# zkeown/mlx-audio-primitives

Measured on AMD Instinct MI355X. Metric: mel-spectrogram frames/sec (n_fft=2048, n_mels=128), higher is better.
Workload: dtype f32

## Files before the change

mlx-audio-primitives_amd/csrc/kernels_mel2048.h:

```cpp
#pragma once
#include <type_traits>
#include "kernels_wave.h"

#define APM_WAVES 8
#define APM_RUN 8
#define APM_PARTIAL_OFF 1152


#define APM_REG_WIN 1
#define APM_REG_TW1 2
#define APM_REG_TW2 4
#define APM_REG_SPLIT 8
#define APM_REGS (APM_REG_WIN | APM_REG_SPLIT)

template <int REGS>
AP_DEV void apm_forward(const ap_float2 (&x)[16], const ap_float2 (&w)[16], ap_float2 *X, const ap_float2 *TW1,
                        const ap_float2 *tw2row, const ap_float2 (&t1r)[16], const ap_float2 (&t2r)[16],
                        const ApwLane &c, const ApmLane &m) {
    const int lane = c.lane;
    ap_float2 v[16];
    if (REGS & APM_REG_TW1) {
        ApButterfly<16>::run_weighted(x, w, v);
#pragma unroll
        for (int k = 1; k < 16; ++k) v[k] = ap_mul_fw(v[k], t1r[k]);
    } else {
        ap_float2 t1[16];
#pragma unroll
        for (int k = 1; k < 16; ++k) t1[k] = TW1[k * 64 + lane];
        ApButterfly<16>::run_weighted(x, w, v);
#pragma unroll
        for (int k = 1; k < 16; ++k) v[k] = ap_mul_fw(v[k], t1[k]);
    }
    {
        const int a = lane & 3, bq = lane >> 2;
#pragma unroll
        for (int k = 0; k < 16; ++k) X[APW_T1(k * 4 + a) + bq] = v[k];
    }
    AP_WAVE_SYNC();
    ap_float2 t2[16];
#pragma unroll
    for (int i = 0; i < 16; ++i) v[i] = X[APW_T1(lane) + i];
    if (!(REGS & APM_REG_TW2)) {
#pragma unroll
        for (int cc = 1; cc < 16; ++cc) t2[cc] = tw2row[cc];
    }
    AP_WAVE_SYNC();
    ApButterfly<16>::run(v);
    v[0] = ap_scale(v[0], m.sg);
#pragma unroll
    for (int cc = 1; cc < 16; ++cc) v[cc] = ap_mul_fw(v[cc], (REGS & APM_REG_TW2) ? t2r[cc] : t2[cc]);
    apm_quad_radix4(v, m);
#pragma unroll
    for (int cc = 0; cc < 16; ++cc) X[apw_zidx(c.k1p + 16 * cc + 256 * c.qd)] = v[cc];
    AP_WAVE_SYNC();
}

template <int REGS>
AP_DEV void apm_split(const ap_float2 *X, const ApwLane &c, const ap_float2 (&wsp)[8], ap_float2 (&xk)[8],
                      ap_float2 (&xm)[8], ap_float2 &zh) {
    ap_float2 zk[8], zm[8];
#pragma unroll
    for (int r = 0; r < 8; ++r) {
        const int k = c.lane + 64 * r;
        zk[r] = X[apw_zidx(k)];
        zm[r] = X[apw_zidx((APW_NC - k) & (APW_NC - 1))];
    }
    zh = X[apw_zidx(APW_NC / 2)];
    AP_WAVE_SYNC();
#pragma unroll
    for (int r = 0; r < 8; ++r) {
        const ap_float2 a = ap_add_conj(zk[r], zm[r]);
        const ap_float2 d = ap_sub_conj(zk[r], zm[r]);
        const ap_float2 w = (REGS & APM_REG_SPLIT) ? wsp[r]
                                                   : (r == 0 ? c.tws0h : ap_mul_bw_c(c.tws0h, APW_C32(r), APW_S32(r)));
        const ap_float2 u = ap_mul_fw(d, w);
        xk[r] = ap_fma_add_mi(a, c.half, u);
        xm[r] = ap_fma_sub_mi(a, c.half, u);
    }
}

#ifdef AP_DIAG_STAMPS
#define AP_DIAG_BEGIN() unsigned long long ap_dt0, ap_dr0; \
    asm volatile("s_memtime %0\n\ts_memrealtime %1\n\ts_waitcnt lgkmcnt(0)" : "=s"(ap_dt0), "=s"(ap_dr0)::"memory")
#define AP_DIAG_END(widx) do { unsigned long long ap_dt1, ap_dr1; \
    asm volatile("s_memtime %0\n\ts_memrealtime %1\n\ts_waitcnt lgkmcnt(0)" : "=s"(ap_dt1), "=s"(ap_dr1)::"memory"); \
    if ((threadIdx.x & 63) == 0 && (widx) < 256 * 16) { ap_diag_stamps[4 * (widx)] = ap_dt1 - ap_dt0; ap_diag_stamps[4 * (widx) + 1] = ap_dr1 - ap_dr0; ap_diag_stamps[4 * (widx) + 2] = ap_dr0; ap_diag_stamps[4 * (widx) + 3] = ap_dr1; } } while (0)
#else
#define AP_DIAG_BEGIN() do {} while (0)
#define AP_DIAG_END(widx) do {} while (0)
#endif

#ifdef AP_HOST_EMU
#define AP_FAIR_SHARE(wave, nw, f) do {} while (0)
#else
#define AP_FAIR_SHARE(wave, nw, f)                                   \
    do {                                                             \
        if ((wave) >= (nw) / 2 + ((nw) > 8 ? 2 : 0)) {               \
            if ((f) & 1) __builtin_amdgcn_s_setprio(1);              \
            else __builtin_amdgcn_s_setprio(0);                      \
        } else if ((nw) > 8 && (wave) >= 4) {                        \
            if ((f) & 1) __builtin_amdgcn_s_setprio(0);              \
            else __builtin_amdgcn_s_setprio(1);                      \
        }                                                            \
    } while (0)
#endif

template <int PMODE, int NPASS, int HOPJ, int IN16 = 0, int NW = APM_WAVES, int REGS = APM_REGS>
__global__ void __launch_bounds__(64 * NW, NW / 4) ap_mel2048_run_kernel(ApMelWaveParams P) {
    static_assert(IN16 != 1 || (REGS & APM_REG_WIN), "the PCM scale rides on the register-resident window");
    const int tid = threadIdx.x;
    const int lane = tid & 63;
    const int wave = AP_UNIFORM(tid >> 6);
    ap_float2 *X = reinterpret_cast<ap_float2 *>(ap_smem) + wave * APW_X_COMPLEX;
    ap_float2 *TW2 = reinterpret_cast<ap_float2 *>(ap_smem + P.off_tw2);
    const ap_float2 *TW1 = reinterpret_cast<const ap_float2 *>(ap_smem + P.off_tw1);
    const ap_float2 *WIN = reinterpret_cast<const ap_float2 *>(ap_smem + P.off_win);
    const ap_float4 *WQ = reinterpret_cast<const ap_float4 *>(ap_smem + P.off_wq);
    float *pp = reinterpret_cast<float *>(X);
    float *partial = pp + APM_PARTIAL_OFF;
    const int M = P.n_mels;

    {
        const int nt = 64 * NW;
        ap_float4 *wq = reinterpret_cast<ap_float4 *>(ap_smem + P.off_wq);
        for (int i = tid; i < P.n_quads; i += nt) wq[i] = reinterpret_cast<const ap_float4 *>(P.quads)[i];
        apw_fill_tables(TW2, reinterpret_cast<ap_float2 *>(ap_smem + P.off_tw1),
                        reinterpret_cast<ap_float2 *>(ap_smem + P.off_win), P.tw, P.window, tid, nt);
    }
    AP_LDS_BARRIER();
    const ApwLane lc = apw_lane_init(lane, TW2, P.tw);
    const ApmLane lm = apm_lane_init(lane);
    ap_float2 winr[16], t1r[16], t2r[16], wsp[8];
#pragma unroll
    for (int j = 0; j < 16; ++j) {
        winr[j] = (REGS & APM_REG_WIN) ? reinterpret_cast<const ap_float2 *>(P.window)[lane + 64 * j] : ap_mk(0.0f, 0.0f);
        if (IN16 == 1) winr[j] = ap_scale(winr[j], 1.0f / 32768.0f);
        t1r[j] = (REGS & APM_REG_TW1) ? P.tw[(2 * lane * j) & 2047] : ap_mk(0.0f, 0.0f);
        t2r[j] = (REGS & APM_REG_TW2) ? ap_scale(P.tw[32 * (lane & 3) * j], lm.sg) : ap_mk(0.0f, 0.0f);
    }
#pragma unroll
    for (int r = 0; r < 8; ++r)
        wsp[r] = (REGS & APM_REG_SPLIT) ? ap_scale(P.tw[lane + 64 * r], 0.5f) : ap_mk(0.0f, 0.0f);
    const ap_float4 *pqa[NPASS], *pqb[NPASS];
    float *sa[NPASS], *sb[NPASS];
    float fz[NPASS];
#pragma unroll
    for (int ps = 0; ps < NPASS; ++ps) {
        const int pi = lane + 64 * ps;
        ap_int4 pd;
        pd.x = P.n_slots; pd.y = 0; pd.z = P.n_slots; pd.w = 0;
        if (pi < P.n_parts) pd = reinterpret_cast<const ap_int4 *>(P.parts)[pi];
        pqa[ps] = reinterpret_cast<const ap_float4 *>(pp) + pd.y;
        pqb[ps] = reinterpret_cast<const ap_float4 *>(pp) + pd.w;
        sa[ps] = partial + pd.x;
        sb[ps] = partial + (pd.z < 0 ? P.n_slots : pd.z);
        fz[ps] = pd.z < 0 ? 1.0f : 0.0f;
    }
    int rs0[2], cnt[2];
#pragma unroll
    for (int i = 0; i < 2; ++i) {
        const int row = lane + 64 * i;
        rs0[i] = row < M ? P.rowstart[row] : 0;
        cnt[i] = row < M ? P.rowstart[row + 1] - rs0[i] : 0;
    }
    AP_LDS_BARRIER();

    const int64_t worker = (int64_t)blockIdx.x * NW + wave;
    const int64_t n_workers = (int64_t)gridDim.x * NW;
    const int64_t n_frames = P.n_clips * P.T;
    const int64_t f_lo = n_frames * worker / n_workers, f_hi = n_frames * (worker + 1) / n_workers;
    const int Ti = (int)P.T;
    float vmax = -INFINITY;
    AP_DIAG_BEGIN();
    if (f_lo < f_hi) {
        int64_t b = f_lo / P.T;
        int t = (int)(f_lo - b * P.T);
        const int16_t *y16 = reinterpret_cast<const int16_t *>(P.y);
        ApClip clip = ap_clip_make(P.y + (IN16 == 1 ? 0 : b * P.L), IN16 == 1 ? 0 : P.L);
        ApClip16 clip16 = ap_clip16_make(y16 + (IN16 == 1 ? b * P.L : 0), IN16 == 1 ? P.L : 0);
        auto ld2 = [&](int64_t bb, int base, int p) -> ap_float2 {
            if (IN16 == 1) return ap_clip16_load2(clip16, p);
            if (IN16 == 2 && !(base >= 0 && (int64_t)base + 2 * APW_NC <= P.L)) {
                const float *yb = P.y + bb * P.L;
                return ap_mk(ap_load_padded(yb, P.L, p, P.pad_mode), ap_load_padded(yb, P.L, p + 1, P.pad_mode));
            }
            return ap_clip_load2(clip, p);
        };
        constexpr int U = HOPJ == 4 ? 4 : 1;
        ap_float2 raw[16];
        auto load_frame = [&](int tt, auto rot_tag) {
            constexpr int ROT = decltype(rot_tag)::value;
            const int base = tt * P.hop - P.pad;
#pragma unroll
            for (int j = 0; j < 16; ++j) {
                const int p = base + 2 * (lane + 64 * j);
                raw[(j + HOPJ * ROT) & 15] = ld2(b, base, p);
            }
        };
        const int r0 = U == 4 ? (t & 3) : 0;
        if (r0 == 1) load_frame(t, std::integral_constant<int, 1 % U>());
        else if (r0 == 2) load_frame(t, std::integral_constant<int, 2 % U>());
        else if (r0 == 3) load_frame(t, std::integral_constant<int, 3 % U>());
        else load_frame(t, std::integral_constant<int, 0>());
        float acc0[APM_RUN], acc1[APM_RUN];
#pragma unroll
        for (int i = 0; i < APM_RUN; ++i) { acc0[i] = 0.0f; acc1[i] = 0.0f; }
        int nrun = 0, half = U == 4 ? ((t >> 2) & 1) : 0;
        int64_t f = f_lo;

        auto frame = [&](auto rot_tag) -> bool {
            constexpr int ROT = decltype(rot_tag)::value;
            constexpr int NROT = (ROT + 1) % U;
            AP_FAIR_SHARE(wave, NW, f);
            const bool clip_ends = t + 1 == Ti;
            const bool more = f + 1 < f_hi;
            {
                ap_float2 xs[16], ws[16];
#pragma unroll
                for (int j = 0; j < 16; ++j) xs[j] = raw[(j + HOPJ * ROT) & 15];
                if (REGS & APM_REG_WIN) {
#pragma unroll
                    for (int j = 0; j < 16; ++j) ws[j] = winr[j];
                } else {
#pragma unroll
                    for (int j = 0; j < 16; ++j) ws[j] = WIN[lane + 64 * j];
                }
                AP_SCHED_FENCE();
                apm_forward<REGS>(xs, ws, X, TW1, lc.tw2row, t1r, t2r, lc, lm);
            }
            AP_SCHED_FENCE();
            if (more) {
                if (clip_ends) {
                    if (IN16 == 1) clip16 = ap_clip16_make(y16 + (b + 1) * P.L, P.L);
                    else clip = ap_clip_make(P.y + (b + 1) * P.L, P.L);
                }
                const int base = (clip_ends ? 0 : t + 1) * P.hop - P.pad;
#pragma unroll
                for (int j = 16 - HOPJ; j < 16; ++j) {
                    const int p = base + 2 * (lane + 64 * j);
                    raw[(j + HOPJ * NROT) & 15] = ld2(clip_ends ? b + 1 : b, base, p);
                }
                if (HOPJ == 0 || clip_ends) {
#pragma unroll
                    for (int j = 0; j < 16 - HOPJ; ++j) {
                        const int p = base + 2 * (lane + 64 * j);
                        raw[(j + HOPJ * NROT) & 15] = ld2(clip_ends ? b + 1 : b, base, p);
                    }
                }
            }
            AP_SCHED_FENCE();
            {
                ap_float2 xk[8], xm[8], zh;
                apm_split<REGS>(X, lc, wsp, xk, xm, zh);
#pragma unroll
                for (int r = 0; r < 8; ++r) {
                    const int k = lane + 64 * r;
                    pp[k] = apw_pow2x<PMODE>(xk[r].x, xk[r].y, P.power);
                    pp[APW_NC - k] = apw_pow2x<PMODE>(xm[r].x, xm[r].y, P.power);
                }
                if (lane == 0) pp[APW_NC / 2] = apw_pow2x<PMODE>(zh.x, zh.y, P.power);
            }
            AP_WAVE_SYNC();
#pragma unroll
            for (int ps = 0; ps < NPASS; ++ps) {
                const ap_float4 *wq = WQ + 256 * ps + lane;
                ap_float4 w[4], q[4];
#pragma unroll
                for (int i = 0; i < 4; ++i) w[i] = wq[64 * i];
                q[0] = pqa[ps][0]; q[1] = pqa[ps][1]; q[2] = pqb[ps][0]; q[3] = pqb[ps][1];
                float acc[2] = {0.0f, 0.0f};
#pragma unroll
                for (int i = 0; i < 4; ++i) {
                    acc[i >> 1] = fmaf(w[i].x, q[i].x, acc[i >> 1]);
                    acc[i >> 1] = fmaf(w[i].y, q[i].y, acc[i >> 1]);
                    acc[i >> 1] = fmaf(w[i].z, q[i].z, acc[i >> 1]);
                    acc[i >> 1] = fmaf(w[i].w, q[i].w, acc[i >> 1]);
                }
                *sa[ps] = fmaf(fz[ps], acc[1], acc[0]);
                *sb[ps] = acc[1];
            }
            AP_WAVE_SYNC();
            float sum2[2];
#pragma unroll
            for (int i = 0; i < 2; ++i) {
                const float p0 = partial[rs0[i]], p1 = partial[rs0[i] + 1], p2 = partial[rs0[i] + 2],
                            p3 = partial[rs0[i] + 3];
                float sum = cnt[i] > 0 ? p0 : 0.0f;
                sum += cnt[i] > 1 ? p1 : 0.0f;
                sum += cnt[i] > 2 ? p2 : 0.0f;
                sum += cnt[i] > 3 ? p3 : 0.0f;
                sum2[i] = sum;
                vmax = fmaxf(vmax, cnt[i] > 0 ? sum : vmax);
            }
            int pos;
            if (U == 1) {
#pragma unroll
                for (int i = 0; i < APM_RUN - 1; ++i) { acc0[i] = acc0[i + 1]; acc1[i] = acc1[i + 1]; }
                acc0[APM_RUN - 1] = sum2[0];
                acc1[APM_RUN - 1] = sum2[1];
                pos = APM_RUN - 1;
            } else {
                if (half) { acc0[4 + ROT] = sum2[0]; acc1[4 + ROT] = sum2[1]; }
                else { acc0[ROT] = sum2[0]; acc1[ROT] = sum2[1]; }
                pos = 4 * half + ROT;
            }
            ++nrun;
            AP_WAVE_SYNC();
            if ((U == 1 ? nrun == APM_RUN : pos == APM_RUN - 1) || clip_ends || !more) {
                const int first = pos - nrun + 1;
                float *ob = P.out + b * (int64_t)M * P.Ts + (t - nrun + 1);
#pragma unroll
                for (int i = 0; i < 2; ++i) {
                    const int row = lane + 64 * i;
                    if (row < M) {
                        float *dst = ob + (int64_t)row * P.Ts;
                        const float *src = i == 0 ? acc0 : acc1;
                        if (nrun == APM_RUN) {
                            ap_rsp_f4u lo, hi;
                            lo.x = src[0]; lo.y = src[1]; lo.z = src[2]; lo.w = src[3];
                            hi.x = src[4]; hi.y = src[5]; hi.z = src[6]; hi.w = src[7];
                            *reinterpret_cast<ap_rsp_f4u *>(dst) = lo;
                            *reinterpret_cast<ap_rsp_f4u *>(dst + 4) = hi;
                        } else {
#pragma unroll
                            for (int g = 0; g < APM_RUN; ++g)
                                if (g >= first && g <= pos) dst[g - first] = src[g];
                        }
                    }
                }
                nrun = 0;
            }
            if (clip_ends) { t = 0; ++b; } else { ++t; }
            ++f;
            return more;
        };
        if (U == 1) {
            while (frame(std::integral_constant<int, 0>())) {}
        } else {
            int skip = r0;
            for (;;) {
                if (skip <= 0 && !frame(std::integral_constant<int, 0>())) break;
                if (skip <= 1 && !frame(std::integral_constant<int, 1 % U>())) break;
                if (skip <= 2 && !frame(std::integral_constant<int, 2 % U>())) break;
                if (!frame(std::integral_constant<int, 3 % U>())) break;
                skip = 0;
                half ^= 1;
            }
        }
    }
    AP_DIAG_END((int)worker);
    if (P.max_key) {
        AP_WAVE_SYNC();
        partial[lane] = vmax;
        AP_WAVE_SYNC();
        if (lane == 0) {
            float m = partial[0];
            for (int i = 1; i < 64; ++i) m = fmaxf(m, partial[i]);
            ap_atomic_max_u32(P.max_key, ap_fkey(m));
        }
    }
}

#ifdef AP_HOST_EMU
AP_DEV float apm_lane_xor(float x, int mask) { return emu_lane_xor(x, mask); }
AP_DEV float apm_lane_up(float x, int d, int lane) { return emu_lane_perm(x, lane - d); }
#else
AP_DEV float apm_lane_xor(float x, int mask) { return __shfl_xor(x, mask, 64); }
AP_DEV float apm_lane_up(float x, int d, int lane) { return __shfl_up(x, d, 64); }
#endif
AP_DEV float apm_wave_sum(float x) {
#pragma unroll
    for (int off = 32; off > 0; off >>= 1) x += apm_lane_xor(x, off);
    return x;
}

template <int PMODE, int HOPJ, int FLAT, int PGEN = 0, int NW = APM_WAVES, int REGS = APM_REGS>
__global__ void __launch_bounds__(64 * NW, NW / 4) ap_spec2048_run_kernel(ApSpecWaveParams P) {
    const int tid = threadIdx.x;
    const int lane = tid & 63;
    const int wave = AP_UNIFORM(tid >> 6);
    ap_float2 *X = reinterpret_cast<ap_float2 *>(ap_smem) + wave * APW_X_COMPLEX;
    ap_float2 *TW2 = reinterpret_cast<ap_float2 *>(ap_smem + P.off_tw2);
    const ap_float2 *TW1 = reinterpret_cast<const ap_float2 *>(ap_smem + P.off_tw1);
    const ap_float2 *WIN = reinterpret_cast<const ap_float2 *>(ap_smem + P.off_win);
    float *pp = reinterpret_cast<float *>(X);
    apw_fill_tables(TW2, reinterpret_cast<ap_float2 *>(ap_smem + P.off_tw1),
                    reinterpret_cast<ap_float2 *>(ap_smem + P.off_win), P.tw, P.window, tid, 64 * NW);
    AP_LDS_BARRIER();
    const ApwLane lc = apw_lane_init(lane, TW2, P.tw);
    const ApmLane lm = apm_lane_init(lane);
    ap_float2 winr[16], t1r[16], t2r[16], wsp[8];
#pragma unroll
    for (int j = 0; j < 16; ++j) {
        winr[j] = (REGS & APM_REG_WIN) ? reinterpret_cast<const ap_float2 *>(P.window)[lane + 64 * j] : ap_mk(0.0f, 0.0f);
        t1r[j] = (REGS & APM_REG_TW1) ? P.tw[(2 * lane * j) & 2047] : ap_mk(0.0f, 0.0f);
        t2r[j] = (REGS & APM_REG_TW2) ? ap_scale(P.tw[32 * (lane & 3) * j], lm.sg) : ap_mk(0.0f, 0.0f);
    }
#pragma unroll
    for (int r = 0; r < 8; ++r)
        wsp[r] = (REGS & APM_REG_SPLIT) ? ap_scale(P.tw[lane + 64 * r], 0.5f) : ap_mk(0.0f, 0.0f);
    float fk[17];
#pragma unroll
    for (int i = 0; i < 16; ++i) fk[i] = P.freq[16 * lane + i];
    fk[16] = lane == 63 ? P.freq[APW_NC] : 0.0f;
    AP_LDS_BARRIER();

    const int64_t worker = (int64_t)blockIdx.x * NW + wave;
    const int64_t n_workers = (int64_t)gridDim.x * NW;
    const int64_t n_frames = P.n_clips * P.T;
    const int64_t f_lo = n_frames * worker / n_workers, f_hi = n_frames * (worker + 1) / n_workers;
    const int Ti = (int)P.T;
    if (f_lo >= f_hi) return;
    int64_t b = f_lo / P.T;
    int t = (int)(f_lo - b * P.T);
    ApClip clip = ap_clip_make(P.y + b * P.L, P.L);
    constexpr int U = HOPJ == 4 ? 4 : 1;
    ap_float2 raw[16];
    auto load_frame = [&](int tt, auto rot_tag) {
        constexpr int ROT = decltype(rot_tag)::value;
        const int base = tt * P.hop - P.pad;
#pragma unroll
        for (int j = 0; j < 16; ++j) raw[(j + HOPJ * ROT) & 15] = ap_clip_load2(clip, base + 2 * (lane + 64 * j));
    };
    load_frame(t, std::integral_constant<int, 0>());
    int64_t f = f_lo;
    const float F_all = (float)(APW_NC + 1);

    auto frame = [&](auto rot_tag) -> bool {
        constexpr int ROT = decltype(rot_tag)::value;
        constexpr int NROT = (ROT + 1) % U;
        const bool clip_ends = t + 1 == Ti;
        const bool more = f + 1 < f_hi;
        {
            ap_float2 xs[16], ws[16];
#pragma unroll
            for (int j = 0; j < 16; ++j) xs[j] = raw[(j + HOPJ * ROT) & 15];
            if (REGS & APM_REG_WIN) {
#pragma unroll
                for (int j = 0; j < 16; ++j) ws[j] = winr[j];
            } else {
#pragma unroll
                for (int j = 0; j < 16; ++j) ws[j] = WIN[lane + 64 * j];
            }
            AP_SCHED_FENCE();
            apm_forward<REGS>(xs, ws, X, TW1, lc.tw2row, t1r, t2r, lc, lm);
        }
        AP_SCHED_FENCE();
        if (more) {
            if (clip_ends) clip = ap_clip_make(P.y + (b + 1) * P.L, P.L);
            const int base = (clip_ends ? 0 : t + 1) * P.hop - P.pad;
#pragma unroll
            for (int j = 16 - HOPJ; j < 16; ++j)
                raw[(j + HOPJ * NROT) & 15] = ap_clip_load2(clip, base + 2 * (lane + 64 * j));
            if (HOPJ == 0 || clip_ends) {
#pragma unroll
                for (int j = 0; j < 16 - HOPJ; ++j)
                    raw[(j + HOPJ * NROT) & 15] = ap_clip_load2(clip, base + 2 * (lane + 64 * j));
            }
        }
        AP_SCHED_FENCE();
        {
            ap_float2 xk[8], xm[8], zh;
            apm_split<REGS>(X, lc, wsp, xk, xm, zh);
#pragma unroll
            for (int r = 0; r < 8; ++r) {
                const int k = lane + 64 * r;
                pp[k] = apw_pow2x<PMODE>(xk[r].x, xk[r].y, P.power);
                pp[APW_NC - k] = apw_pow2x<PMODE>(xm[r].x, xm[r].y, P.power);
            }
            if (lane == 0) pp[APW_NC / 2] = apw_pow2x<PMODE>(zh.x, zh.y, P.power);
        }
        AP_WAVE_SYNC();
        float v[17];
#pragma unroll
        for (int q4 = 0; q4 < 4; ++q4) {
            const ap_float4 a = reinterpret_cast<const ap_float4 *>(pp)[4 * lane + q4];
            v[4 * q4] = a.x; v[4 * q4 + 1] = a.y; v[4 * q4 + 2] = a.z; v[4 * q4 + 3] = a.w;
        }
        v[16] = lane == 63 ? pp[APW_NC] : 0.0f;
        AP_WAVE_SYNC();
        float s0 = 0.0f, s1 = 0.0f;
#pragma unroll
        for (int i = 0; i < 17; ++i) { s0 += v[i]; s1 = fmaf(fk[i], v[i], s1); }
        const float tot = apm_wave_sum(s0), tf = apm_wave_sum(s1);
        const float cen = tf / (tot + 1e-10f);
        const int64_t o = b * P.T + t;
        if (P.centroid && lane == 0) P.centroid[o] = cen;
        if (FLAT) {
            float sl = 0.0f, sa = 0.0f;
#pragma unroll
            for (int i = 0; i < 17; ++i) {
                const float c = fmaxf(v[i], P.amin);
                if (i < 16 || lane == 63) { sl += logf(c); sa += c; }
            }
            const float tl = apm_wave_sum(sl), ta = apm_wave_sum(sa);
            if (P.flatness && lane == 0) P.flatness[o] = expf(tl / F_all) / (ta / F_all + 1e-10f);
        }
        if (P.bandwidth) {
            float dev = 0.0f;
#pragma unroll
            for (int i = 0; i < 17; ++i) {
                const float d = fabsf(fk[i] - cen);
                dev = fmaf(v[i], PGEN ? powf(d, P.p) : d * d, dev);
            }
            float w = apm_wave_sum(dev);
            if (P.norm) w = w / (tot + 1e-10f);
            if (lane == 0) P.bandwidth[o] = PGEN ? powf(w, 1.0f / P.p) : sqrtf(w);
        }
        if (P.rolloff) {
            float incl = s0;
#pragma unroll
            for (int d = 1; d < 64; d <<= 1) {
                const float up = apm_lane_up(incl, d, lane);
                if (lane >= d) incl += up;
            }
            const float before = incl - s0;
            const float thr = tot * P.roll_percent;
            const bool mine = (before + s0 >= thr) && (lane == 0 || before < thr);
            float run = before, fsel = lane == 63 ? fk[16] : fk[15];
            bool found = false;
#pragma unroll
            for (int i = 0; i < 17; ++i) {
                if (i < 16 || lane == 63) {
                    run += v[i];
                    if (!found && run >= thr) { found = true; fsel = fk[i]; }
                }
            }
            float cand = (mine && found) ? fsel : INFINITY;
#pragma unroll
            for (int off = 32; off > 0; off >>= 1) cand = fminf(cand, apm_lane_xor(cand, off));
            const float last = apm_lane_xor(fk[16], 63);
            if (lane == 0) P.rolloff[o] = !(tot >= thr) ? fk[0] : (cand < INFINITY ? cand : last);
        }
        if (clip_ends) { t = 0; ++b; } else { ++t; }
        ++f;
        return more;
    };
    if (U == 1) {
        while (frame(std::integral_constant<int, 0>())) {}
    } else {
        for (;;) {
            if (!frame(std::integral_constant<int, 0>())) break;
            if (!frame(std::integral_constant<int, 1 % U>())) break;
            if (!frame(std::integral_constant<int, 2 % U>())) break;
            if (!frame(std::integral_constant<int, 3 % U>())) break;
        }
    }
}
```

mlx-audio-primitives_amd/csrc/kernels_wave.h:

```cpp
#pragma once
#include "ap_wave_params.h"
#include "fft_lds.h"
#include "kernels_generic.h"

#if defined(AP_DIAG_STAMPS) && !defined(AP_HOST_EMU)
__device__ unsigned long long ap_diag_stamps[4 * 256 * 16];
#endif

#define APW_C32(r) ((float)__builtin_cos(6.283185307179586476925 * (r) / 32.0))
#define APW_S32(r) ((float)__builtin_sin(6.283185307179586476925 * (r) / 32.0))

#ifdef AP_HOST_EMU
#define AP_WAVE_SYNC() emu_wave_sync()
#define AP_SCHED_FENCE() do {} while (0)
#define AP_PIN(x) do {} while (0)
#else
#define AP_SCHED_FENCE() __builtin_amdgcn_sched_barrier(0)
#define AP_PIN(x) asm volatile("" : "+v"(x))
#define AP_WAVE_SYNC()                                          \
    do {                                                        \
        __builtin_amdgcn_fence(__ATOMIC_RELEASE, "wavefront");  \
        __builtin_amdgcn_wave_barrier();                        \
        __builtin_amdgcn_fence(__ATOMIC_ACQUIRE, "wavefront");  \
    } while (0)

AP_DEV float ap_quad_xor1(float x) {
    return __builtin_bit_cast(float, __builtin_amdgcn_mov_dpp(__builtin_bit_cast(int, x), 0xB1, 0xF, 0xF, true));
}
AP_DEV float ap_quad_xor2(float x) {
    return __builtin_bit_cast(float, __builtin_amdgcn_mov_dpp(__builtin_bit_cast(int, x), 0x4E, 0xF, 0xF, true));
}
#endif


AP_DEV int apw_zidx(int k) { return k + 4 * (k >> 8); }

template <int PMODE>
AP_DEV float apw_pow2x(float re, float im, float power) {
    const float p2 = re * re + im * im;
    if (PMODE == 2) return p2;
    if (PMODE == 1) return sqrtf(p2);
    return powf(sqrtf(p2), power);
}

#ifdef AP_HOST_EMU
#define AP_UNIFORM(x) (x)
struct ApClip { const float *base; int64_t n; };
AP_DEV ApClip ap_clip_make(const float *base, int64_t n) { ApClip c; c.base = base; c.n = n; return c; }
AP_DEV float ap_clip_load(const ApClip &c, int64_t idx) { return (idx >= 0 && idx < c.n) ? c.base[idx] : 0.0f; }
AP_DEV ap_float2 ap_clip_load2(const ApClip &c, int64_t idx) { return ap_mk(ap_clip_load(c, idx), ap_clip_load(c, idx + 1)); }
struct ApClip16 { const int16_t *base; int64_t n; };
AP_DEV ApClip16 ap_clip16_make(const int16_t *base, int64_t n) { ApClip16 c; c.base = base; c.n = n; return c; }
AP_DEV ap_float2 ap_clip16_load2(const ApClip16 &c, int64_t idx) {
    return ap_mk((idx >= 0 && idx < c.n) ? (float)c.base[idx] : 0.0f,
                 (idx + 1 >= 0 && idx + 1 < c.n) ? (float)c.base[idx + 1] : 0.0f);
}
struct ApOutBuf { char *base; int64_t bytes; };
AP_DEV ApOutBuf ap_outbuf_make(void *base, int64_t bytes) { ApOutBuf o; o.base = (char *)base; o.bytes = bytes; return o; }
AP_DEV ap_float2 ap_outbuf_load2(const ApOutBuf &o, unsigned lane_bytes, unsigned uniform_bytes) {
    const uint64_t off = (uint64_t)lane_bytes + uniform_bytes;
    if (lane_bytes < 0x80000000u && off + 8 <= (uint64_t)o.bytes) return *reinterpret_cast<const ap_float2 *>(o.base + off);
    return ap_mk(0.0f, 0.0f);
}
AP_DEV void ap_outbuf_store2(const ApOutBuf &o, unsigned lane_bytes, unsigned uniform_bytes, ap_float2 v) {
    const uint64_t off = (uint64_t)lane_bytes + uniform_bytes;
    if (lane_bytes < 0x80000000u && off + 8 <= (uint64_t)o.bytes) *reinterpret_cast<ap_float2 *>(o.base + off) = v;
}
#else
#define AP_UNIFORM(x) __builtin_amdgcn_readfirstlane(x)
typedef __amdgpu_buffer_rsrc_t ApClip;
AP_DEV ApClip ap_clip_make(const float *base, int64_t n) {
    return __builtin_amdgcn_make_buffer_rsrc(const_cast<float *>(base), 0, (int)(n * 4), 0x00020000);
}
AP_DEV float ap_clip_load(ApClip c, int64_t idx) {
    int off = (int)(idx * 4);
    AP_PIN(off);
    return __builtin_bit_cast(float, __builtin_amdgcn_raw_buffer_load_b32(c, off, 0, 0));
}
AP_DEV ap_float2 ap_clip_load2(ApClip c, int idx) {
    typedef int ap_i2 __attribute__((ext_vector_type(2)));
    return __builtin_bit_cast(ap_float2, __builtin_bit_cast(ap_i2, __builtin_amdgcn_raw_buffer_load_b64(c, idx * 4, 0, 0)));
}
typedef __amdgpu_buffer_rsrc_t ApOutBuf;
AP_DEV ApOutBuf ap_outbuf_make(void *base, int64_t bytes) {
    return __builtin_amdgcn_make_buffer_rsrc(base, 0, (int)bytes, 0x00020000);
}
AP_DEV ap_float2 ap_outbuf_load2(ApOutBuf o, unsigned lane_bytes, unsigned uniform_bytes) {
    typedef int ap_i2 __attribute__((ext_vector_type(2)));
    return __builtin_bit_cast(ap_float2, __builtin_amdgcn_raw_buffer_load_b64(o, (int)lane_bytes, (int)uniform_bytes, 0));
}
AP_DEV void ap_outbuf_store2(ApOutBuf o, unsigned lane_bytes, unsigned uniform_bytes, ap_float2 v) {
    typedef int ap_i2 __attribute__((ext_vector_type(2)));
    __builtin_amdgcn_raw_buffer_store_b64(__builtin_bit_cast(ap_i2, v), o, (int)lane_bytes, (int)uniform_bytes, 0);
}
typedef __amdgpu_buffer_rsrc_t ApClip16;
AP_DEV ApClip16 ap_clip16_make(const int16_t *base, int64_t n) {
    return __builtin_amdgcn_make_buffer_rsrc(const_cast<int16_t *>(base), 0, (int)(n * 2), 0x00020000);
}
AP_DEV ap_float2 ap_clip16_load2(ApClip16 c, int idx) {
    int off = idx * 2;
    AP_PIN(off);
    const int d = __builtin_amdgcn_raw_buffer_load_b32(c, off, 0, 0);
    return ap_mk((float)(short)(d & 0xFFFF), (float)(d >> 16));
}
#endif


struct ApwLane {
    int lane, qa, qd, k1p;
    float s1, s2;
    ap_float2 rotw;
    const ap_float2 *tw2row;
    ap_float2 tws0h;
    ap_float2 half, halfc;
};

AP_DEV ApwLane apw_lane_init(int lane, const ap_float2 *TW2, const ap_float2 *tw) {
    ApwLane c;
    c.lane = lane;
    c.qa = lane & 3;
    c.s1 = c.qa < 2 ? 1.0f : -1.0f;
    c.s2 = (c.qa & 1) ? -1.0f : 1.0f;
    c.rotw = c.qa == 3 ? ap_mk(0.0f, 1.0f) : ap_mk(1.0f, 0.0f);
    c.qd = ((c.qa & 1) << 1) | (c.qa >> 1);
    c.k1p = lane >> 2;
    c.tw2row = TW2 + c.qa * 17;
    c.tws0h = ap_scale(tw[lane], 0.5f);
    c.half = ap_mk(0.5f, 0.5f);
    c.halfc = ap_mk(0.5f, -0.5f);
    return c;
}

AP_DEV void apw_fill_tables(ap_float2 *tw2, ap_float2 *tw1, ap_float2 *win, const ap_float2 *tw,
                            const float *window, int tid, int nt) {
    if (tid < 64) {
        const int a = tid >> 4;
        tw2[a * 17 + (tid & 15)] = ap_scale(tw[32 * a * (tid & 15)], (a == 1 || a == 2) ? -1.0f : 1.0f);
    }
    for (int i = tid; i < 16 * 64; i += nt) tw1[i] = tw[2 * (i & 63) * (i >> 6)];
    for (int i = tid; i < APW_NC; i += nt) win[i] = reinterpret_cast<const ap_float2 *>(window)[i];
}

struct ApmLane {
    float c1, c2;
    float sg;
    bool rot;
};

AP_DEV ApmLane apm_lane_init(int lane) {
    ApmLane m;
    const int qa = lane & 3;
    const float s1 = qa < 2 ? 1.0f : -1.0f, s2 = (qa & 1) ? -1.0f : 1.0f;
    m.c1 = -s1;
    m.c2 = -s2;
    m.sg = s1 * s2;
    m.rot = qa == 3;
    return m;
}

#ifdef AP_HOST_EMU
AP_DEV void apm_quad8(ap_float2 *v, const ApmLane &m) {
    for (int i = 0; i < 8; ++i) {
        v[i].x = v[i].x + m.c1 * ap_quad_xor2(v[i].x);
        v[i].y = v[i].y + m.c1 * ap_quad_xor2(v[i].y);
    }
    for (int i = 0; i < 8; ++i) {
        const float rx = v[i].x, ry = v[i].y;
        v[i].x = m.rot ? ry : rx;
        v[i].y = m.rot ? -rx : ry;
    }
    for (int i = 0; i < 8; ++i) {
        v[i].x = v[i].x + m.c2 * ap_quad_xor1(v[i].x);
        v[i].y = v[i].y + m.c2 * ap_quad_xor1(v[i].y);
    }
}
#else
#define APM_ROT(ix, iy, nx, ny)                            \
    "v_cndmask_b32 %" #nx ", %" #ix ", %" #iy ", %34\n\t"  \
    "v_cndmask_b32 %" #ny ", %" #iy ", -%" #ix ", %34\n\t"
#define APM_S2N(i) "v_fmac_f32_dpp %" #i ", %" #i ", %33 quad_perm:[1,0,3,2] row_mask:0xf bank_mask:0xf\n\t"
#define APM_S1N(i) "v_fmac_f32_dpp %" #i ", %" #i ", %32 quad_perm:[2,3,0,1] row_mask:0xf bank_mask:0xf\n\t"
AP_DEV void apm_quad8(ap_float2 *v, const ApmLane &m) {
    ap_float2 n[8];
    const unsigned long long rot_mask = 0x8888888888888888ull;
    asm volatile(
        "s_nop 1\n\t"
        APM_S1N(0) APM_S1N(1) APM_S1N(2) APM_S1N(3) APM_S1N(4) APM_S1N(5) APM_S1N(6) APM_S1N(7)
        APM_S1N(8) APM_S1N(9) APM_S1N(10) APM_S1N(11) APM_S1N(12) APM_S1N(13) APM_S1N(14) APM_S1N(15)
        APM_ROT(0, 1, 16, 17) APM_ROT(2, 3, 18, 19) APM_ROT(4, 5, 20, 21) APM_ROT(6, 7, 22, 23)
        APM_ROT(8, 9, 24, 25) APM_ROT(10, 11, 26, 27) APM_ROT(12, 13, 28, 29) APM_ROT(14, 15, 30, 31)
        APM_S2N(16) APM_S2N(17) APM_S2N(18) APM_S2N(19) APM_S2N(20) APM_S2N(21) APM_S2N(22) APM_S2N(23)
        APM_S2N(24) APM_S2N(25) APM_S2N(26) APM_S2N(27) APM_S2N(28) APM_S2N(29) APM_S2N(30) APM_S2N(31)
        : "+v"(v[0].x), "+v"(v[0].y), "+v"(v[1].x), "+v"(v[1].y), "+v"(v[2].x), "+v"(v[2].y), "+v"(v[3].x), "+v"(v[3].y),
          "+v"(v[4].x), "+v"(v[4].y), "+v"(v[5].x), "+v"(v[5].y), "+v"(v[6].x), "+v"(v[6].y), "+v"(v[7].x), "+v"(v[7].y),
          "=&v"(n[0].x), "=&v"(n[0].y), "=&v"(n[1].x), "=&v"(n[1].y), "=&v"(n[2].x), "=&v"(n[2].y), "=&v"(n[3].x), "=&v"(n[3].y),
          "=&v"(n[4].x), "=&v"(n[4].y), "=&v"(n[5].x), "=&v"(n[5].y), "=&v"(n[6].x), "=&v"(n[6].y), "=&v"(n[7].x), "=&v"(n[7].y)
        : "v"(m.c1), "v"(m.c2), "s"(rot_mask));
#pragma unroll
    for (int i = 0; i < 8; ++i) v[i] = n[i];
}
#undef APM_S1N
#undef APM_S2N
#undef APM_ROT
#endif

AP_DEV void apm_quad_radix4(ap_float2 (&v)[16], const ApmLane &m) {
    apm_quad8(&v[0], m);
    apm_quad8(&v[8], m);
}

AP_DEV void apw_butterfly16_tight(ap_float2 (&v)[16]) {
    ap_float2 a[4][4];
#pragma unroll
    for (int r = 0; r < 4; ++r) {
        a[r][0] = v[r]; a[r][1] = v[r + 4]; a[r][2] = v[r + 8]; a[r][3] = v[r + 12];
        ap_fft4(a[r][0], a[r][1], a[r][2], a[r][3]);
        AP_SCHED_FENCE();
    }
    const float C1 = 0.92387953251128675613f, S1 = 0.38268343236508977173f;
    const float H = 0.70710678118654752440f;
#pragma unroll
    for (int p = 0; p < 4; ++p) {
        if (p == 1) {
            a[1][1] = ap_mul_fw_c(a[1][1], C1, S1);
            a[2][1] = ap_mul_fw_c(a[2][1], H, H);
            a[3][1] = ap_mul_fw_c(a[3][1], S1, C1);
        } else if (p == 2) {
            a[1][2] = ap_mul_fw_c(a[1][2], H, H);
            a[3][2] = ap_mul_fw_c(a[3][2], -H, H);
        } else if (p == 3) {
            a[1][3] = ap_mul_fw_c(a[1][3], S1, C1);
            a[2][3] = ap_mul_fw_c(a[2][3], -H, H);
            a[3][3] = ap_mul_fw_c(a[3][3], -C1, -S1);
        }
        if (p == 2) ap_fft4_a2mi(a[0][p], a[1][p], a[2][p], a[3][p]);
        else ap_fft4(a[0][p], a[1][p], a[2][p], a[3][p]);
        v[p] = a[0][p]; v[p + 4] = a[1][p]; v[p + 8] = a[2][p]; v[p + 12] = a[3][p];
        AP_SCHED_FENCE();
    }
}

#ifndef AP_HOST_EMU
#define AP_PRIO(n) __builtin_amdgcn_s_setprio(n)
#else
#define AP_PRIO(n) do {} while (0)
#endif

template <bool TO_LDS = true, bool TIGHT = false, bool PRIO = false>
AP_DEV void apw_forward(ap_float2 (&v)[16], ap_float2 *X, const ap_float2 *TW1, const ApwLane &c) {
    const int lane = c.lane;
    if (TIGHT) {
        apw_butterfly16_tight(v);
#pragma unroll
        for (int h = 0; h < 2; ++h) {
            ap_float2 t1[8];
#pragma unroll
            for (int k = 0; k < 8; ++k) if (8 * h + k) t1[k] = TW1[(8 * h + k) * 64 + lane];
#pragma unroll
            for (int k = 0; k < 8; ++k) if (8 * h + k) v[8 * h + k] = ap_mul_fw(v[8 * h + k], t1[k]);
            AP_SCHED_FENCE();
        }
    } else {
        ap_float2 t1[16];
#pragma unroll
        for (int k = 1; k < 16; ++k) t1[k] = TW1[k * 64 + lane];
        ApButterfly<16>::run(v);
#pragma unroll
        for (int k = 1; k < 16; ++k) v[k] = ap_mul_fw(v[k], t1[k]);
    }
    if (PRIO) AP_PRIO(2);
    {
        const int a = lane & 3, bq = lane >> 2;
#pragma unroll
        for (int k = 0; k < 16; ++k) X[APW_T1(k * 4 + a) + bq] = v[k];
    }
    AP_WAVE_SYNC();
    ap_float2 t2[16];
#pragma unroll
    for (int i = 0; i < 16; ++i) v[i] = X[APW_T1(lane) + i];
    if (!TIGHT) {
#pragma unroll
        for (int cc = 1; cc < 16; ++cc) t2[cc] = c.tw2row[cc];
    }
    AP_WAVE_SYNC();
    const ApmLane m = apm_lane_init(lane);
    if (TIGHT) {
        AP_SCHED_FENCE();
        apw_butterfly16_tight(v);
        v[0] = ap_scale(v[0], m.sg);
#pragma unroll
        for (int h = 0; h < 2; ++h) {
#pragma unroll
            for (int k = 0; k < 8; ++k) if (8 * h + k) t2[k] = c.tw2row[8 * h + k];
#pragma unroll
            for (int k = 0; k < 8; ++k) if (8 * h + k) v[8 * h + k] = ap_mul_fw(v[8 * h + k], t2[k]);
            AP_SCHED_FENCE();
        }
    } else {
        ApButterfly<16>::run(v);
        v[0] = ap_scale(v[0], m.sg);
#pragma unroll
        for (int cc = 1; cc < 16; ++cc) v[cc] = ap_mul_fw(v[cc], t2[cc]);
    }
    if (PRIO) AP_PRIO(1);
    apm_quad_radix4(v, m);
    if (TO_LDS) {
#pragma unroll
        for (int cc = 0; cc < 16; ++cc) X[apw_zidx(c.k1p + 16 * cc + 256 * c.qd)] = v[cc];
        AP_WAVE_SYNC();
    }
}

template <bool CONJ>
AP_DEV void apw_split(const ap_float2 *X, const ApwLane &c, ap_float2 (&xk)[8], ap_float2 (&xm)[8],
                      ap_float2 &zh) {
    ap_float2 zk[8], zm[8];
#pragma unroll
    for (int r = 0; r < 8; ++r) {
        const int k = c.lane + 64 * r;
        zk[r] = X[apw_zidx(k)];
        zm[r] = X[apw_zidx((APW_NC - k) & (APW_NC - 1))];
    }
    zh = X[apw_zidx(APW_NC / 2)];
    AP_WAVE_SYNC();
#pragma unroll
    for (int r = 0; r < 8; ++r) {
        const ap_float2 a = ap_add_conj(zk[r], zm[r]);
        const ap_float2 d = ap_sub_conj(zk[r], zm[r]);
        const ap_float2 w = r == 0 ? c.tws0h : ap_mul_bw_c(c.tws0h, APW_C32(r), APW_S32(r));
        const ap_float2 u = ap_mul_fw(d, w);
        xk[r] = ap_fma_add_mi(a, c.half, u);
        xm[r] = CONJ ? ap_fma_sub_swap(a, c.halfc, u) : ap_fma_sub_mi(a, c.half, u);
    }
}

template <int PMODE, int PADGEN>
__global__ void __launch_bounds__(64 * APW_WAVES, 2) ap_mel2048_wave_kernel(ApMelWaveParams P) {
    const int tid = threadIdx.x;
    const int lane = tid & 63;
    const int wave = AP_UNIFORM(tid >> 6);
    ap_float2 *X = reinterpret_cast<ap_float2 *>(ap_smem) + wave * APW_X_COMPLEX;
    const ap_float2 *TW2 = reinterpret_cast<const ap_float2 *>(ap_smem + P.off_tw2);
    const ap_float2 *TW1 = reinterpret_cast<const ap_float2 *>(ap_smem + P.off_tw1);
    const ap_float2 *WIN = reinterpret_cast<const ap_float2 *>(ap_smem + P.off_win);
    const ap_float4 *WQ = reinterpret_cast<const ap_float4 *>(ap_smem + P.off_wq);
    const ap_int4 *PART = reinterpret_cast<const ap_int4 *>(ap_smem + P.off_parts);
    float *partial = reinterpret_cast<float *>(ap_smem + P.off_partial) + wave * P.partial_stride;
    float *otile = reinterpret_cast<float *>(ap_smem + P.off_otile) + wave * P.otile_stride * APW_G;
    const int M = P.n_mels;

    {
        const int nt = 64 * APW_WAVES;
        ap_float4 *wq = reinterpret_cast<ap_float4 *>(ap_smem + P.off_wq);
        ap_int4 *part = reinterpret_cast<ap_int4 *>(ap_smem + P.off_parts);
        for (int i = tid; i < P.n_quads; i += nt) wq[i] = reinterpret_cast<const ap_float4 *>(P.quads)[i];
        if (P.n_parts > 64 * APW_PASSES)
            for (int i = tid; i < P.n_parts; i += nt) part[i] = reinterpret_cast<const ap_int4 *>(P.parts)[i];
        apw_fill_tables(reinterpret_cast<ap_float2 *>(ap_smem + P.off_tw2),
                        reinterpret_cast<ap_float2 *>(ap_smem + P.off_tw1),
                        reinterpret_cast<ap_float2 *>(ap_smem + P.off_win), P.tw, P.window, tid, nt);
    }
    const ApwLane lc = apw_lane_init(lane, TW2, P.tw);
    float *pp = reinterpret_cast<float *>(X);
    ap_int4 mypart[APW_PASSES];
#pragma unroll
    for (int ps = 0; ps < APW_PASSES; ++ps) {
        const int pi = lane + 64 * ps;
        mypart[ps].x = 0; mypart[ps].y = 0; mypart[ps].z = 0; mypart[ps].w = 0;
        if (pi < P.n_parts) mypart[ps] = reinterpret_cast<const ap_int4 *>(P.parts)[pi];
    }
    int rs0[2], rs1[2];
#pragma unroll
    for (int i = 0; i < 2; ++i) {
        const int row = lane + 64 * i;
        rs0[i] = row < M ? P.rowstart[row] : 0;
        rs1[i] = row < M ? P.rowstart[row + 1] : 0;
    }
    AP_LDS_BARRIER();

    const int64_t worker = (int64_t)blockIdx.x * APW_WAVES + wave;
    const int64_t n_workers = (int64_t)gridDim.x * APW_WAVES;
    const int64_t n_frames = P.n_clips * P.T;
    const int64_t f_lo = n_frames * worker / n_workers, f_hi = n_frames * (worker + 1) / n_workers;
    float vmax = -INFINITY;
#ifdef AP_DIAG_STAMPS
    unsigned long long ap_dt0, ap_dr0;
    asm volatile("s_memtime %0\n\ts_memrealtime %1\n\ts_waitcnt lgkmcnt(0)" : "=s"(ap_dt0), "=s"(ap_dr0)::"memory");
#endif
    ap_float2 raw[16];
    auto load_frame = [&](int64_t f) {
        const int64_t b = f / P.T;
        const int64_t t = f - b * P.T;
        const float *yb = P.y + b * P.L;
        const ApClip clip = ap_clip_make(yb, P.L);
        const int64_t base = t * (int64_t)P.hop - P.pad;
        const bool inside = !PADGEN || (base >= 0 && base + 2 * APW_NC <= P.L);
        if (inside) {
#pragma unroll
            for (int j = 0; j < 16; ++j) {
                const int64_t p = base + 2 * (lane + 64 * j);
                raw[j] = ap_clip_load2(clip, (int)p);
            }
        } else {
#pragma unroll
            for (int j = 0; j < 16; ++j) {
                const int64_t p = base + 2 * (lane + 64 * j);
                raw[j] = ap_mk(ap_load_padded(yb, P.L, p, P.pad_mode), ap_load_padded(yb, P.L, p + 1, P.pad_mode));
            }
        }
    };
    auto next_frame = [&](int64_t f) {
        const int64_t b = f / P.T;
        const int64_t t = f - b * P.T;
        if (PADGEN || t == 0 || P.hopj == 0) { load_frame(f); return; }
        const ApClip clip = ap_clip_make(P.y + b * P.L, P.L);
        const int64_t base = t * (int64_t)P.hop - P.pad;
#define APW_SHIFT_LOAD(S)                                                                    \
        {                                                                                    \
            _Pragma("unroll") for (int j = 0; j < 16 - (S); ++j) raw[j] = raw[j + (S)];      \
            _Pragma("unroll") for (int j = 16 - (S); j < 16; ++j) {                           \
                const int64_t p = base + 2 * (lane + 64 * j);                                \
                raw[j] = ap_clip_load2(clip, (int)p);            \
            }                                                                                \
        }
        if (P.hopj == 4) APW_SHIFT_LOAD(4)
        else if (P.hopj == 2) APW_SHIFT_LOAD(2)
        else APW_SHIFT_LOAD(8)
#undef APW_SHIFT_LOAD
    };
    if (f_lo < f_hi) load_frame(f_lo);

    for (int64_t f = f_lo; f < f_hi;) {
        const int64_t b = f / P.T;
        const int64_t t0 = f - b * P.T;
        int64_t run = P.T - t0;
        if (run > APW_G) run = APW_G;
        if (run > f_hi - f) run = f_hi - f;
        const int Gt = (int)run;
        float *ob = P.out + b * (int64_t)M * P.T + t0;

// ... 460 lines not shown
```

Baseline: 586.9 million.

## Fold final radix-4 FFT stage into split via per-lane bin-pair mapping

Removes the cross-lane quad radix-4 stage and sign-scaled twiddles from the forward FFT. Stage-2 outputs are instead stored in a padded group layout, and each lane loads 4 float4 pairs, does local radix-4 butterflies, and directly owns conjugate bin pairs for the real-FFT split. Split twiddles are precomputed per lane from a packed lane-permutation table. The aim is to cut DPP/cross-lane work and use wider LDS reads, at the cost of more complex indexing and a possible change in bank-conflict behaviour.

```diff
diff --git a/mlx-audio-primitives_amd/csrc/kernels_mel2048.h b/mlx-audio-primitives_amd/csrc/kernels_mel2048.h
--- a/mlx-audio-primitives_amd/csrc/kernels_mel2048.h
+++ b/mlx-audio-primitives_amd/csrc/kernels_mel2048.h
@@ -5,7 +5,6 @@
 #define APM_WAVES 8
 #define APM_RUN 8
 #define APM_PARTIAL_OFF 1152
-
 
 #define APM_REG_WIN 1
 #define APM_REG_TW1 2
@@ -13,10 +12,30 @@
 #define APM_REG_SPLIT 8
 #define APM_REGS (APM_REG_WIN | APM_REG_SPLIT)
 
+AP_DEV int apm_gidx(int g) { return 4 * g + 2 * (g >> 3); }
+
+struct ApmPairLane {
+    int L, lp;
+    bool l0;
+    int rd[4];
+};
+
+AP_DEV ApmPairLane apm_pair_lane_init(int lane) {
+    ApmPairLane p;
+    p.L = (int)((0xE311825200ull >> (5 * ((lane >> 2) & 7))) & 31) + (lane & 3) + (lane & 32);
+    p.l0 = p.L == 0;
+    p.lp = p.l0 ? 128 : p.L;
+    p.rd[0] = apm_gidx(p.L);
+    p.rd[1] = apm_gidx(p.L + 64);
+    p.rd[2] = apm_gidx(192 - p.L);
+    p.rd[3] = apm_gidx(256 - p.lp);
+    return p;
+}
+
 template <int REGS>
 AP_DEV void apm_forward(const ap_float2 (&x)[16], const ap_float2 (&w)[16], ap_float2 *X, const ap_float2 *TW1,
                         const ap_float2 *tw2row, const ap_float2 (&t1r)[16], const ap_float2 (&t2r)[16],
-                        const ApwLane &c, const ApmLane &m) {
+                        const ApwLane &c) {
     const int lane = c.lane;
     ap_float2 v[16];
     if (REGS & APM_REG_TW1) {
@@ -46,37 +65,56 @@
     }
     AP_WAVE_SYNC();
     ApButterfly<16>::run(v);
-    v[0] = ap_scale(v[0], m.sg);
 #pragma unroll
     for (int cc = 1; cc < 16; ++cc) v[cc] = ap_mul_fw(v[cc], (REGS & APM_REG_TW2) ? t2r[cc] : t2[cc]);
-    apm_quad_radix4(v, m);
-#pragma unroll
-    for (int cc = 0; cc < 16; ++cc) X[apw_zidx(c.k1p + 16 * cc + 256 * c.qd)] = v[cc];
+    const int wb = apm_gidx(c.k1p) + (lane & 3);
+#pragma unroll
+    for (int cc = 0; cc < 16; ++cc) X[wb + 68 * cc] = v[cc];
     AP_WAVE_SYNC();
 }
 
-template <int REGS>
-AP_DEV void apm_split(const ap_float2 *X, const ApwLane &c, const ap_float2 (&wsp)[8], ap_float2 (&xk)[8],
-                      ap_float2 (&xm)[8], ap_float2 &zh) {
-    ap_float2 zk[8], zm[8];
-#pragma unroll
-    for (int r = 0; r < 8; ++r) {
-        const int k = c.lane + 64 * r;
-        zk[r] = X[apw_zidx(k)];
-        zm[r] = X[apw_zidx((APW_NC - k) & (APW_NC - 1))];
-    }
-    zh = X[apw_zidx(APW_NC / 2)];
+AP_DEV void apm_pair_bins(const ApmPairLane &p, int (&k)[8]) {
+    k[0] = p.L; k[1] = p.L + 256; k[2] = 512 - p.lp; k[3] = 256 - p.lp;
+    k[4] = p.L + 64; k[5] = p.L + 320; k[6] = 448 - p.L; k[7] = 192 - p.L;
+}
+
+AP_DEV void apm_split_twiddles(const ApmPairLane &p, const ap_float2 *tw, ap_float2 (&wsp)[8]) {
+    int k[8];
+    apm_pair_bins(p, k);
+#pragma unroll
+    for (int i = 0; i < 8; ++i) wsp[i] = ap_scale(tw[k[i]], 0.5f);
+}
+
+template <int PMODE>
+AP_DEV void apm_split(const ap_float2 *X, float *pp, const ApmPairLane &p, const ap_float2 (&wsp)[8],
+                      const ApwLane &c, float power) {
+    ap_float2 z[4][4];
+#pragma unroll
+    for (int s = 0; s < 4; ++s) {
+        const ap_float4 *src = reinterpret_cast<const ap_float4 *>(X + p.rd[s]);
+        const ap_float4 lo = src[0], hi = src[1];
+        z[s][0] = ap_mk(lo.x, lo.y); z[s][1] = ap_mk(lo.z, lo.w);
+        z[s][2] = ap_mk(hi.x, hi.y); z[s][3] = ap_mk(hi.z, hi.w);
+    }
     AP_WAVE_SYNC();
 #pragma unroll
-    for (int r = 0; r < 8; ++r) {
-        const ap_float2 a = ap_add_conj(zk[r], zm[r]);
-        const ap_float2 d = ap_sub_conj(zk[r], zm[r]);
-        const ap_float2 w = (REGS & APM_REG_SPLIT) ? wsp[r]
-                                                   : (r == 0 ? c.tws0h : ap_mul_bw_c(c.tws0h, APW_C32(r), APW_S32(r)));
-        const ap_float2 u = ap_mul_fw(d, w);
-        xk[r] = ap_fma_add_mi(a, c.half, u);
-        xm[r] = ap_fma_sub_mi(a, c.half, u);
-    }
+    for (int s = 0; s < 4; ++s) ap_fft4(z[s][0], z[s][1], z[s][2], z[s][3]);
+    const ap_float2 zk[8] = {z[0][0], z[0][1], z[3][1], z[3][0], z[1][0], z[1][1], z[2][1], z[2][0]};
+    const ap_float2 zm[8] = {p.l0 ? z[0][0] : z[3][3], p.l0 ? z[0][3] : z[3][2], p.l0 ? z[3][2] : z[0][2],
+                             p.l0 ? z[3][3] : z[0][3], z[2][3], z[2][2], z[1][2], z[1][3]};
+    int k[8];
+    apm_pair_bins(p, k);
+#pragma unroll
+    for (int i = 0; i < 8; ++i) {
+        const ap_float2 a = ap_add_conj(zk[i], zm[i]);
+        const ap_float2 d = ap_sub_conj(zk[i], zm[i]);
+        const ap_float2 u = ap_mul_fw(d, wsp[i]);
+        const ap_float2 xk = ap_fma_add_mi(a, c.half, u);
+        const ap_float2 xm = ap_fma_sub_mi(a, c.half, u);
+        pp[k[i]] = apw_pow2x<PMODE>(xk.x, xk.y, power);
+        pp[APW_NC - k[i]] = apw_pow2x<PMODE>(xm.x, xm.y, power);
+    }
+    if (p.l0) pp[APW_NC / 2] = apw_pow2x<PMODE>(z[0][2].x, z[0][2].y, power);
 }
 
 #ifdef AP_DIAG_STAMPS
@@ -124,23 +162,21 @@
         const int nt = 64 * NW;
         ap_float4 *wq = reinterpret_cast<ap_float4 *>(ap_smem + P.off_wq);
         for (int i = tid; i < P.n_quads; i += nt) wq[i] = reinterpret_cast<const ap_float4 *>(P.quads)[i];
-        apw_fill_tables(TW2, reinterpret_cast<ap_float2 *>(ap_smem + P.off_tw1),
-                        reinterpret_cast<ap_float2 *>(ap_smem + P.off_win), P.tw, P.window, tid, nt);
+        apw_fill_tables<false>(TW2, reinterpret_cast<ap_float2 *>(ap_smem + P.off_tw1),
+                               reinterpret_cast<ap_float2 *>(ap_smem + P.off_win), P.tw, P.window, tid, nt);
     }
     AP_LDS_BARRIER();
     const ApwLane lc = apw_lane_init(lane, TW2, P.tw);
-    const ApmLane lm = apm_lane_init(lane);
+    const ApmPairLane pl = apm_pair_lane_init(lane);
     ap_float2 winr[16], t1r[16], t2r[16], wsp[8];
 #pragma unroll
     for (int j = 0; j < 16; ++j) {
         winr[j] = (REGS & APM_REG_WIN) ? reinterpret_cast<const ap_float2 *>(P.window)[lane + 64 * j] : ap_mk(0.0f, 0.0f);
         if (IN16 == 1) winr[j] = ap_scale(winr[j], 1.0f / 32768.0f);
         t1r[j] = (REGS & APM_REG_TW1) ? P.tw[(2 * lane * j) & 2047] : ap_mk(0.0f, 0.0f);
-        t2r[j] = (REGS & APM_REG_TW2) ? ap_scale(P.tw[32 * (lane & 3) * j], lm.sg) : ap_mk(0.0f, 0.0f);
-    }
-#pragma unroll
-    for (int r = 0; r < 8; ++r)
-        wsp[r] = (REGS & APM_REG_SPLIT) ? ap_scale(P.tw[lane + 64 * r], 0.5f) : ap_mk(0.0f, 0.0f);
+        t2r[j] = (REGS & APM_REG_TW2) ? P.tw[32 * (lane & 3) * j] : ap_mk(0.0f, 0.0f);
+    }
+    apm_split_twiddles(pl, P.tw, wsp);
     const ap_float4 *pqa[NPASS], *pqb[NPASS];
     float *sa[NPASS], *sb[NPASS];
     float fz[NPASS];
@@ -226,7 +262,7 @@
                     for (int j = 0; j < 16; ++j) ws[j] = WIN[lane + 64 * j];
                 }
                 AP_SCHED_FENCE();
-                apm_forward<REGS>(xs, ws, X, TW1, lc.tw2row, t1r, t2r, lc, lm);
+                apm_forward<REGS>(xs, ws, X, TW1, lc.tw2row, t1r, t2r, lc);
             }
             AP_SCHED_FENCE();
             if (more) {
@@ -249,17 +285,7 @@
                 }
             }
             AP_SCHED_FENCE();
-            {
-                ap_float2 xk[8], xm[8], zh;
-                apm_split<REGS>(X, lc, wsp, xk, xm, zh);
-#pragma unroll
-                for (int r = 0; r < 8; ++r) {
-                    const int k = lane + 64 * r;
-                    pp[k] = apw_pow2x<PMODE>(xk[r].x, xk[r].y, P.power);
-                    pp[APW_NC - k] = apw_pow2x<PMODE>(xm[r].x, xm[r].y, P.power);
-                }
-                if (lane == 0) pp[APW_NC / 2] = apw_pow2x<PMODE>(zh.x, zh.y, P.power);
-            }
+            apm_split<PMODE>(X, pp, pl, wsp, lc, P.power);
             AP_WAVE_SYNC();
 #pragma unroll
             for (int ps = 0; ps < NPASS; ++ps) {
@@ -384,21 +410,19 @@
     const ap_float2 *TW1 = reinterpret_cast<const ap_float2 *>(ap_smem + P.off_tw1);
     const ap_float2 *WIN = reinterpret_cast<const ap_float2 *>(ap_smem + P.off_win);
     float *pp = reinterpret_cast<float *>(X);
-    apw_fill_tables(TW2, reinterpret_cast<ap_float2 *>(ap_smem + P.off_tw1),
-                    reinterpret_cast<ap_float2 *>(ap_smem + P.off_win), P.tw, P.window, tid, 64 * NW);
+    apw_fill_tables<false>(TW2, reinterpret_cast<ap_float2 *>(ap_smem + P.off_tw1),
+                           reinterpret_cast<ap_float2 *>(ap_smem + P.off_win), P.tw, P.window, tid, 64 * NW);
     AP_LDS_BARRIER();
     const ApwLane lc = apw_lane_init(lane, TW2, P.tw);
-    const ApmLane lm = apm_lane_init(lane);
+    const ApmPairLane pl = apm_pair_lane_init(lane);
     ap_float2 winr[16], t1r[16], t2r[16], wsp[8];
 #pragma unroll
     for (int j = 0; j < 16; ++j) {
         winr[j] = (REGS & APM_REG_WIN) ? reinterpret_cast<const ap_float2 *>(P.window)[lane + 64 * j] : ap_mk(0.0f, 0.0f);
         t1r[j] = (REGS & APM_REG_TW1) ? P.tw[(2 * lane * j) & 2047] : ap_mk(0.0f, 0.0f);
-        t2r[j] = (REGS & APM_REG_TW2) ? ap_scale(P.tw[32 * (lane & 3) * j], lm.sg) : ap_mk(0.0f, 0.0f);
-    }
-#pragma unroll
-    for (int r = 0; r < 8; ++r)
-        wsp[r] = (REGS & APM_REG_SPLIT) ? ap_scale(P.tw[lane + 64 * r], 0.5f) : ap_mk(0.0f, 0.0f);
+        t2r[j] = (REGS & APM_REG_TW2) ? P.tw[32 * (lane & 3) * j] : ap_mk(0.0f, 0.0f);
+    }
+    apm_split_twiddles(pl, P.tw, wsp);
     float fk[17];
 #pragma unroll
     for (int i = 0; i < 16; ++i) fk[i] = P.freq[16 * lane + i];
@@ -443,7 +467,7 @@
                 for (int j = 0; j < 16; ++j) ws[j] = WIN[lane + 64 * j];
             }
             AP_SCHED_FENCE();
-            apm_forward<REGS>(xs, ws, X, TW1, lc.tw2row, t1r, t2r, lc, lm);
+            apm_forward<REGS>(xs, ws, X, TW1, lc.tw2row, t1r, t2r, lc);
         }
         AP_SCHED_FENCE();
         if (more) {
@@ -459,17 +483,7 @@
             }
         }
         AP_SCHED_FENCE();
-        {
-            ap_float2 xk[8], xm[8], zh;
-            apm_split<REGS>(X, lc, wsp, xk, xm, zh);
-#pragma unroll
-            for (int r = 0; r < 8; ++r) {
-                const int k = lane + 64 * r;
-                pp[k] = apw_pow2x<PMODE>(xk[r].x, xk[r].y, P.power);
-                pp[APW_NC - k] = apw_pow2x<PMODE>(xm[r].x, xm[r].y, P.power);
-            }
-            if (lane == 0) pp[APW_NC / 2] = apw_pow2x<PMODE>(zh.x, zh.y, P.power);
-        }
+        apm_split<PMODE>(X, pp, pl, wsp, lc, P.power);
         AP_WAVE_SYNC();
         float v[17];
 #pragma unroll
diff --git a/mlx-audio-primitives_amd/csrc/kernels_wave.h b/mlx-audio-primitives_amd/csrc/kernels_wave.h
--- a/mlx-audio-primitives_amd/csrc/kernels_wave.h
+++ b/mlx-audio-primitives_amd/csrc/kernels_wave.h
@@ -131,11 +131,12 @@
     return c;
 }
 
+template <bool QUAD_SIGNS = true>
 AP_DEV void apw_fill_tables(ap_float2 *tw2, ap_float2 *tw1, ap_float2 *win, const ap_float2 *tw,
                             const float *window, int tid, int nt) {
     if (tid < 64) {
         const int a = tid >> 4;
-        tw2[a * 17 + (tid & 15)] = ap_scale(tw[32 * a * (tid & 15)], (a == 1 || a == 2) ? -1.0f : 1.0f);
+        tw2[a * 17 + (tid & 15)] = ap_scale(tw[32 * a * (tid & 15)], (QUAD_SIGNS && (a == 1 || a == 2)) ? -1.0f : 1.0f);
     }
     for (int i = tid; i < 16 * 64; i += nt) tw1[i] = tw[2 * (i & 63) * (i >> 6)];
     for (int i = tid; i < APW_NC; i += nt) win[i] = reinterpret_cast<const ap_float2 *>(window)[i];
```

Measured after the change: 613.0 million, median of 6. 1.04x the previous value.
